# cliangyu/video-diffusion

Measured on AMD Instinct MI355X. Metric: denoise-steps/sec, higher is better.
Workload: dtype f32

## Files before the change

include/vd_amd.h:

```cpp
#ifndef VD_AMD_H
#define VD_AMD_H
#ifdef __cplusplus
extern "C" {
#endif

typedef struct vd_config {
    int image_size;
    int num_channels;
    int num_res_blocks;
    int num_heads;
    int T;
    int n_attention_ds;
    int attention_ds[8];
    int use_scale_shift_norm;
    int use_spatial_encoding;
    int use_frame_encoding;
    int enforce_position_invariance;
    int use_rpe_net;
    int allow_interactions_between_padding;
    float rp_alpha, rp_beta, rp_gamma;
    int time_embed_mult;
    int cond_emb_type;
    int learn_sigma;
} vd_config;
// ... 141 lines not shown
int vd_op_conv_split(const float* src0, int Cin, int nfr, int Hs, int Ws, int stride, const void* w_split, const float* bias,
                     const float* res, float* out, int Cout, void* stream);
int vd_pack_conv3_wino_split(const float* host_oihw, unsigned short* host_out, int O, int I);
int vd_op_conv_wino_split(const float* src0, int Cin, int nfr, int Hs, int Ws, int ups, const void* w_split, const float* bias,
                          const float* res, const float* fbias, int fbias_ld, float* out, int Cout, double* gn_part,
                          void* stream);
int vd_op_conv_wino_act(const float* src0, const float* src1, int C0, int Cin, int nfr, int Hs, int Ws, const void* w_split, const float* bias,
                        const float* affA, const float* affB, const float* res, float* out, int Cout, double* gn_part, void* stream);
int vd_conv_wino_act_ok(int nfr, int H, int Cin, int Cout);
int vd_pack_conv3_wino_ups(const float* host_oihw, unsigned short* host_out, int O, int I);
int vd_conv_ups_stats_split(int Hs);
int vd_op_conv_wino_ups(const float* src0, int Cin, int nfr, int Hs, const void* w_ups, const float* bias, float* out, int Cout,
                        double* gn_part, void* stream);
int vd_op_linear_split(const float* a, int M, int K, const void* w_split, const float* bias, const float* res, int act,
                       float* out, int N, void* stream);
int vd_op_linear_split_stats(const float* a, int M, int K, const void* w_split, const float* bias, const float* res, int act,
                             float* out, int N, int HW, double* gn_part, void* stream);
int vd_linear_stats_split(int M, int N, int HW);
int vd_op_gn_fold(const float* src0, const float* src1, int C0, int C, int nfr, int HW, const float* gamma,
                  const float* beta, const float* film, int film_ld, float* affA, float* affB, void* stream);
int vd_op_affine_apply(const float* x, const float* affA, const float* affB, int nfr, int HW, int C, float* y,
                       void* stream);
int vd_op_affine_act(const float* src0, const float* src1, int C0, int C, const float* affA, const float* affB, int nfr,
                     int HW, int act, float* y, void* stream);
int vd_op_gn_temporal(const float* x, const float* gamma, const float* beta, int B, int T, int HW, int C, float* y,
                      void* stream);
int vd_op_attn_spatial(const float* qkv, int nfr, int L, int C, int heads, float* out, void* stream);
int vd_op_attn_temporal(const float* qkv, const float* Rk, const float* Rq, const float* Rv, const float* mask, int B,
                        int T, int HW, int C, int heads, int allow_pad, float* out, void* stream);
int vd_op_out_conv(const float* x, const float* affA, const float* affB, const float* w_packed, const float* bias,
// ... 59 lines not shown
```

video-diffusion_amd/_lib.py:

```python
import ctypes
import os
import subprocess

_HERE = os.path.dirname(os.path.abspath(__file__))
_CSRC = os.path.join(_HERE, "csrc")
SO_PATH = os.path.join(_HERE, "libvdamd.so")
SOURCES = ["igemm.hip", "conv_wino.hip", "conv_wino_r64.hip", "conv_wino_z128.hip", "gemm_frag.hip", "gemm_split.hip", "split_pack.hip", "norm.hip", "backward.hip", "attn_spatial.hip", "attn_temporal.hip", "attn_temporal_long.hip", "misc.hip", "engine.hip", "lpips.hip", "metrics.hip", "i3d.hip", "conv_cl.hip", "hallway.hip"]
HEADER = os.path.join(os.path.dirname(_HERE), "include", "vd_amd.h")
HEADERS = [os.path.join(_CSRC, "vd_common.h"), os.path.join(_CSRC, "wino_common.h"), os.path.join(_CSRC, "igemm_tile.h"), HEADER]
SOURCE_FLAGS = {"conv_wino_z128.hip": ["-mllvm", "-pragma-unroll-threshold=1000000"]}


def _toolchain():
    hipcc = os.environ.get("HIPCC", "/opt/rocm/bin/hipcc")
    flags = ["--offload-arch=gfx950", "-O3", "-std=c++17", "-fPIC", "-Wno-unused-value"] + \
        os.environ.get("VD_HIPCC_FLAGS", "").split()
    return hipcc, flags


def _sha(*parts):
    import hashlib
    h = hashlib.sha1()
    for p in parts:
        h.update(p if isinstance(p, bytes) else str(p).encode())
# ... 157 lines not shown
    "vd_pack_linear_frag": (_I, [_P, _P, _I, _I]),
    "vd_pack_linear_split": (_I, [_P, _P, _I, _I]),
    "vd_pack_conv3_wino_split": (_I, [_P, _P, _I, _I]),
    "vd_set_model_mean_type": (_I, [_P, _I]),
    "vd_math_mode": (_I, []),
    "vd_split_image_u16": (_L, [_L, _L]),
    "vd_pack_conv3_wino_ups": (_I, [_P, _P, _I, _I]),
    "vd_conv_ups_stats_split": (_I, [_I]),
    "vd_op_conv_wino_ups": (_I, [_P, _I, _I, _I, _P, _P, _P, _I, _P, _P]),
    "vd_op_conv_wino_split": (_I, [_P, _I, _I, _I, _I, _I, _P, _P, _P, _P, _I, _P, _I, _P, _P]),
    "vd_op_conv_wino_act": (_I, [_P, _P, _I, _I, _I, _I, _I, _P, _P, _P, _P, _P, _P, _I, _P, _P]),
    "vd_conv_wino_act_ok": (_I, [_I, _I, _I, _I]),
    "vd_pack_conv3_split": (_I, [_P, _P, _I, _I]),
    "vd_op_conv_split": (_I, [_P, _I, _I, _I, _I, _I, _P, _P, _P, _P, _I, _P]),
    "vd_op_linear_split": (_I, [_P, _I, _I, _P, _P, _P, _I, _P, _I, _P]),
    "vd_op_linear_split_stats": (_I, [_P, _I, _I, _P, _P, _P, _I, _P, _I, _I, _P, _P]),
    "vd_linear_stats_split": (_I, [_I, _I, _I]),
    "vd_op_gn_fold": (_I, [_P, _P, _I, _I, _I, _I, _P, _P, _P, _I, _P, _P, _P]),
    "vd_op_affine_apply": (_I, [_P, _P, _P, _I, _I, _I, _P, _P]),
    "vd_op_affine_act": (_I, [_P, _P, _I, _I, _P, _P, _I, _I, _I, _P, _P]),
    "vd_op_gn_temporal": (_I, [_P, _P, _P, _I, _I, _I, _I, _P, _P]),
    "vd_op_attn_spatial": (_I, [_P, _I, _I, _I, _I, _P, _P]),
    "vd_op_attn_temporal": (_I, [_P, _P, _P, _P, _P, _I, _I, _I, _I, _I, _I, _P, _P]),
    "vd_op_out_conv": (_I, [_P, _P, _P, _P, _P, _I, _I, _I, _I, _I, _P, _P]),
    "vd_op_gn_bwd": (_I, [_P, _P, _I, _I, _P, _P, _P, _P, _I, _I, _I, _P, _P, _I, _P, _I, _P]),
    "vd_op_gn_temporal_bwd": (_I, [_P, _P, _P, _I, _I, _I, _I, _I, _P, _P]),
    "vd_op_attn_temporal_bwd": (_I, [_P, _P, _P, _P, _P, _I, _I, _I, _I, _I, _I, _P, _P, _P]),
    "vd_op_attn_spatial_bwd": (_I, [_P, _I, _I, _I, _I, _P, _P, _P]),
    "vd_op_out_conv_bwd": (_I, [_P, _P, _I, _I, _I, _I, _I, _P, _P]),
    "vd_op_stem_col2im": (_I, [_P, _P, _P, _P, _I, _I, _I, _I, _P, _P]),
# ... 73 lines not shown
```

video-diffusion_amd/csrc/engine.hip:

```cpp
#include <cmath>
#include <cstring>
#include <unordered_map>
#include <vector>

#include "../../include/vd_amd.h"
#include "vd_common.h"

namespace vd {

thread_local std::string g_last_error;
void set_error(const std::string& msg) { g_last_error = msg; }

int launch_frame_t(const int64_t* fidx, int B, int T, int center, float* tv, hipStream_t s);

enum ParamKind { PK_RAW = 0, PK_CONV3, PK_STEM, PK_POSENC, PK_OUTCONV, PK_LINF, PK_CONV3W, PK_CONV3S,
                 PK_CONV3WU };

struct Param {
    std::string name;
    int nd = 0;
    long long shape[4] = {1, 1, 1, 1};
    size_t numel = 0;
    size_t packed = 0;
    size_t off = 0;
// ... 21 lines not shown
struct TapeConv { int type, idx; Tens in, out; };
struct TapePos { Tens in, out; };
struct TapeOp { int kind, i; };
struct Tape {
    std::vector<TapeOp> ops;
    std::vector<TapeRes> res; std::vector<TapeAttn> attn; std::vector<TapeConv> conv; std::vector<TapePos> pos;
    Tens head; float *headA = nullptr, *headB = nullptr, *head_mr = nullptr;
    void clear() { ops.clear(); res.clear(); attn.clear(); conv.clear(); pos.clear(); }
};

static const int CH_MULT_256[] = {1, 1, 2, 2, 4, 4};
static const int CH_MULT_128[] = {1, 1, 2, 3, 4};
static const int CH_MULT_64[] = {1, 2, 3, 4};
static const int CH_MULT_32[] = {1, 2, 2, 2};
static bool split_math() { return math_mode() != MATH_FP32; }

constexpr int STEM_KPAD = 64;

struct Arena {
    char* base = nullptr;
    size_t cap = 0, used = 0, peak = 0;
    bool dry = false, overflow = false;
    template <class Tp> Tp* get(size_t n) {
        size_t bytes = (n * sizeof(Tp) + 255) & ~(size_t)255;
        if (!dry && cap && used + bytes > cap) {
            overflow = true;
            return reinterpret_cast<Tp*>(base);
        }
        char* p = (dry ? reinterpret_cast<char*>(0x1000) : base) + used;
        used += bytes;
// ... 44 lines not shown
};
struct ProfPause {
    bool was = g_prof.on;
    ProfPause() { g_prof.on = false; }
    ~ProfPause() { g_prof.on = was; }
};

static bool act_conv_will_dispatch(const IgemmArgs& g) {
    return g.affA && igemm_kernel(igemm_first_launch(g)) == IK_Z128;
}

static int igemm_p(const IgemmArgs& g, hipStream_t st, int cin_alg = 0) {
    const double taps = (double)g.ksz * g.ksz, cin = cin_alg ? cin_alg : g.Cin;
    const double in_pix = (double)g.nfr * g.Hs * g.Ws;
    const double nz = g.zcount > 1 ? g.zcount : 1;
    const double bytes = nz * 4.0 * (in_pix * cin + (double)g.M * g.Cout * (g.res ? 2 : 1) + taps * cin * g.Cout + (g.side ? in_pix * cin : 0.0));
    const IgemmArgs one = igemm_first_launch(g);
    const IgemmKernel k = igemm_kernel(one);
    const bool wino = k == IK_R64_UPS || k == IK_Z128 || k == IK_R64 || k == IK_WINO;
    const int tile = igemm_tile_class(igemm_sel_M(one), g.Cout);
    int cls;
    switch (k) {
        case IK_R64_UPS: cls = PC_CONV_WINO_R64_UPS; break;
        case IK_Z128: cls = PC_CONV_WINO_Z128; break;
        case IK_R64: cls = PC_CONV_WINO_R64; break;
        case IK_WINO: cls = PC_CONV_WINO; break;
        case IK_SPLIT: cls = gemm_split_tile_class(igemm_sel_M(one), g.Cout) == 4 ? (int)PC_IGEMM_128x192 : tile; break;
        default: cls = tile + (g.ksz == 3 ? (int)PC_CONV_128x128 : 0);
    }
    char tag[56];
    snprintf(tag, sizeof(tag), "M=%d N=%d K=%d k%d s%d%s%s%s", g.M, g.Cout, g.Cin, g.ksz, g.stride, g.ups ? " ups" : "",
             g.affA ? " pro" : (g.act ? " act" : ""), g.res ? " res" : "");
    VD_REQUIRE(g.stats == nullptr || wino || (k == IK_SPLIT && g.stats_hw > 0),
               "GroupNorm partial sums requested from a kernel that has no such epilogue");
    ProfScope ps(cls, nz * 2.0 * g.M * g.Cout * cin * taps, bytes, st, tag);
    return launch_igemm(g, st);
}

static int affine_act(const float* src0, const float* src1, int C0, int C, const float* A, const float* B, int N, int HW,
                      float* y, hipStream_t st) {
    ProfScope ps(PC_ELEMENTWISE, 0.0, 8.0 * N * HW * C, st);
    return launch_affine_act(src0, src1, C0, C, A, B, N, HW, 1, y, st);
}

struct FwdIn {
    int B, T;
    const float *x, *obs_src, *obs, *lat, *km, *t_model;
// ... 511 lines not shown
    const int H = x0.H, HW = H * H;
    const int cin = x0.C + (x1 ? x1->C : 0);
    VD_REQUIRE(cin == r.cin, "ResBlock input channels");
    const float* s1 = x1 ? x1->p : nullptr;
    float *A1 = nullptr, *B1 = nullptr, *A2 = nullptr, *B2 = nullptr, *mr1 = nullptr, *mr2 = nullptr;
    int rc;
    const float* film = film_all + r.film_off;
    IgemmArgs gsk{};
    bool fuse_skip = false;
    if (r.skw >= 0) {
        gsk = conv_args(x0, x1, N, 1, 1, 0);
        set_w(gsk, r.skw); gsk.Cout = r.cout; gsk.ldo = r.cout; gsk.side_hw = HW;
        IgemmArgs one = gsk; one.nfr = std::max(1, std::min(N, igemm_frames_per_launch(gsk)));
        one.M = (g_sel_nfr ? std::max(g_sel_nfr, one.nfr) : one.nfr) * HW;
        one.wfrag = one.wfrag ? one.wfrag : reinterpret_cast<const float*>(0x1000);
        fuse_skip = params[r.skw].kind == PK_LINF && split_math() && gemm_split_side_supported(one);
    }
    const bool fold = !tape;
    const int nsel = g_sel_nfr > N ? g_sel_nfr : N;
    const bool za1 = !tape && params[r.c1w].kind == PK_CONV3W && f16_math() && x0.C % 16 == 0 && conv_wino_z128_act_shape(nsel, H, cin, r.cout);
    if (za1 && !ar.dry) fuse_skip = false;
    const bool fold1 = fold && !fuse_skip;
    const bool za2 = !tape && params[r.c2w].kind == PK_CONV3W && f16_math() && conv_wino_z128_act_shape(nsel, H, r.cout, r.cout);
    if ((!fold1 || za1 || ar.dry) && (rc = gn_fold(x0, x1, N, r.gn1w, r.gn1b, nullptr, 0, st, ar, &A1, &B1, &mr1))) return rc;
    float* h = ar.get<float>((size_t)N * HW * r.cout);
    Tens ht{h, r.cout, H};
    if (params[r.c1w].kind == PK_CONV3W) ht.part = stats_table(ar, N, H, r.cout, &ht.split);
    Tens ot{nullptr, r.cout, H};
    if (params[r.c2w].kind == PK_CONV3W) ot.part = stats_table(ar, N, H, r.cout, &ot.split);
    float* sk_early = fuse_skip ? ar.get<float>((size_t)N * HW * r.cout) : nullptr;
    {
// ... 92 lines not shown
        if (!cfg.use_rpe_net)
            for (int i = 0; i < 3; ++i)
                if ((rc = launch_rpe_table(W(rp[i]->table), fidx, B, T, C, cfg.rp_alpha, cfg.rp_beta, cfg.rp_gamma,
                                           Rall + i * rrows * C, st))) return rc;
        AttnTemporalArgs ta{qkv, R[0], R[1], R[2], amask, o, B, T, HW, C, cfg.num_heads,
                            cfg.allow_interactions_between_padding, scale};
        { const double Fd = C / cfg.num_heads;
          ProfScope ps(PC_ATTN_TEMPORAL, 10.0 * B * HW * cfg.num_heads * T * T * Fd, 16.0 * tok * C + 12.0 * rrows * C, st);
          rc = launch_attn_temporal(ta, st); }
        if (rc) return rc;
        if (!attn_cap_t.empty() && attn_seq < (int)attn_cap_t.size() && attn_cap_t[attn_seq] &&
            (rc = launch_attn_temporal_weights(ta, attn_cap_t[attn_seq], st))) return rc;
        if ((rc = linear(o, (int)tok, C, C, W(a.tp.projw), W(a.tp.projb), 0, xn, xt, st, &xt_t))) return rc;
    }
    float *A = nullptr, *Bf = nullptr, *mrs = nullptr;
    const bool fold = !tape;
    if (!fold && (rc = gn_fold(xt_t, nullptr, N, a.sp.normw, a.sp.normb, nullptr, 0, st, ar, &A, &Bf, &mrs))) return rc;
    float* xn2 = ar.get<float>(tok * C);
    float* qkv2 = ar.get<float>(tok * 3 * C);
    float* o2 = ar.get<float>(tok * C);
    float* xs = ar.get<float>(tok * C);
    Tens xs_t{xs, C, H};
    gemm_stats_table(ar, (int)tok, C, C, &xs_t);
    if (fold && (rc = gn_act(xt_t, nullptr, N, a.sp.normw, a.sp.normb, nullptr, 0, 0, xn2, st, ar))) return rc;
    if (!ar.dry) {
        if (!fold) { ProfScope ps(PC_ELEMENTWISE, 0.0, 8.0 * tok * C, st); rc = launch_affine_apply(xt, A, Bf, N, HW, C, xn2, st); }
        if (rc) return rc;
        if ((rc = linear(xn2, (int)tok, C, 3 * C, W(a.sp.qkvw), W(a.sp.qkvb), 0, nullptr, qkv2, st))) return rc;
        AttnSpatialArgs sa{qkv2, o2, N, HW, C, cfg.num_heads, scale};
        { ProfScope ps(PC_ATTN_SPATIAL, 4.0 * N * (double)HW * HW * C, 16.0 * tok * C, st); rc = launch_attn_spatial(sa, st); }
        if (rc) return rc;
        if (!attn_cap_s.empty() && attn_seq < (int)attn_cap_s.size() && attn_cap_s[attn_seq] &&
            (rc = launch_attn_spatial_weights(sa, attn_cap_s[attn_seq], st))) return rc;
        if ((rc = linear(o2, (int)tok, C, C, W(a.sp.projw), W(a.sp.projb), 0, xn2, xs, st, &xs_t))) return rc;
    }
    *out = xs_t;
    if (!ar.dry) ++attn_seq;
    if (tape) {
        tape->ops.push_back(TapeOp{2, (int)tape->attn.size()});
        tape->attn.push_back(TapeAttn{(int)(&a - attn.data()), x, B, T, xn, qkv, R[0], R[1], R[2], o, xt, A, Bf, mrs, xn2, qkv2, o2, xs, amask});
    }
    return 0;
}

void vd_engine::rpe_group_blocks() {
    if (!rpe_groups.empty()) return;
    for (size_t b = 0; b < attn.size(); ++b) {
        size_t gi = 0;
        while (gi < rpe_groups.size() && rpe_groups[gi].C != attn[b].C) ++gi;
// ... 1339 lines not shown
}

int vd_pack_linear_split(const float* host_w, unsigned short* host_out, int N, int K) {
    VD_REQUIRE(host_w && host_out && N % 32 == 0 && K % 32 == 0, "vd_pack_linear_split: N, K multiples of 32");
    pack_linear_split(host_w, host_out, N, K, N, 0);
    return 0;
}

int vd_op_linear_split(const float* a, int M, int K, const void* w_split, const float* bias, const float* res, int act,
                       float* out, int N, void* stream) {
    IgemmArgs g = linear_args(M, K, N);
    g.src0 = a; g.wfrag = static_cast<const float*>(w_split); g.wsplit = 1; g.bias = bias; g.act = act; g.res = res; g.out = out;
    return launch_igemm(g, static_cast<hipStream_t>(stream));
}

int vd_op_linear_split_stats(const float* a, int M, int K, const void* w_split, const float* bias, const float* res, int act,
                             float* out, int N, int HW, double* gn_part, void* stream) {
    IgemmArgs g = linear_args(M, K, N);
    g.src0 = a; g.wfrag = static_cast<const float*>(w_split); g.wsplit = 1; g.bias = bias; g.act = act; g.res = res; g.out = out;
    VD_REQUIRE(gn_part && HW > 0 && gemm_split_supported(g), "vd_op_linear_split_stats: shape not covered by gemm_split.hip");
    g.stats = gn_part; g.stats_hw = HW; g.stats_split = HW / gemm_split_stats_rows(M, N);
    return launch_igemm(g, static_cast<hipStream_t>(stream));
}

int vd_linear_stats_split(int M, int N, int HW) { return HW / gemm_split_stats_rows(M, N); }

int vd_pack_conv3_wino(const float* host_oihw, float* host_out, int O, int I) {
    VD_REQUIRE(host_oihw && host_out && O % 64 == 0 && I % 16 == 0, "O multiple of 64, I multiple of 16");
    pack_conv3_wino(host_oihw, host_out, O, I);
    return 0;
// ... 206 lines not shown
```

video-diffusion_amd/csrc/gemm_split.hip:

```cpp
#include <cstring>
#include <vector>

#include "vd_common.h"

namespace vd {

typedef __bf16 bf16x4 __attribute__((ext_vector_type(4)));
typedef __bf16 bf16x8 __attribute__((ext_vector_type(8)));
typedef unsigned u32x4 __attribute__((ext_vector_type(4)));
typedef unsigned u32x2 __attribute__((ext_vector_type(2)));

template <bool F16>
__device__ __forceinline__ f32x16 mfma_piece(u32x4 a, u32x4 b, f32x16 c) {
    if constexpr (F16) return __builtin_amdgcn_mfma_f32_32x32x16_f16(__builtin_bit_cast(f16x8, a), __builtin_bit_cast(f16x8, b), c, 0, 0, 0);
    else return __builtin_amdgcn_mfma_f32_32x32x16_bf16(__builtin_bit_cast(bf16x8, a), __builtin_bit_cast(bf16x8, b), c, 0, 0, 0);
}

#ifndef VD_GS_SKIP
#define VD_GS_SKIP 0
#endif
#ifdef VD_GS_TIMING
__device__ unsigned long long g_gs_stamp[8];
#define GS_STAMP(i) do { if (threadIdx.x == 0 && blockIdx.x == gridDim.x / 2 && blockIdx.y == 0) {                        \
        __builtin_amdgcn_sched_barrier(0); g_gs_stamp[i] = __builtin_amdgcn_s_memrealtime(); __builtin_amdgcn_sched_barrier(0); } } while (0)
// ... 8 lines not shown
    if constexpr (F16) {
        p1.x = f16_pack(v.x, v.y); p1.y = f16_pack(v.z, v.w);
        p2.x = f16_pack_scaled(f16_rem_lo(p1.x, v.x), f16_rem_hi(p1.x, v.y));
        p2.y = f16_pack_scaled(f16_rem_lo(p1.y, v.z), f16_rem_hi(p1.y, v.w));
        p3 = p2;
    } else {
        const bf16x4 q1 = __builtin_convertvector(v, bf16x4);
        f32x4 r = v - __builtin_convertvector(q1, f32x4);
        const bf16x4 q2 = __builtin_convertvector(r, bf16x4);
        r = r - __builtin_convertvector(q2, f32x4);
        const bf16x4 q3 = __builtin_convertvector(r, bf16x4);
        p1 = __builtin_bit_cast(u32x2, q1); p2 = __builtin_bit_cast(u32x2, q2); p3 = __builtin_bit_cast(u32x2, q3);
    }
}

template <int BM, int BN, bool ACT, bool CONV, bool F16 = true, bool SIDE = false>
__global__ __launch_bounds__(256, 2) void gemm_split_kernel(IgemmArgs a) {
    constexpr int MI = BM / 64, NI = BN / 64, AR = BM / 32;
    constexpr bool B2R = F16;
    constexpr int RING = NI >= 3 ? 2 : (BM == 64 && BN == 64) ? 6 : 3;
    constexpr int BP = B2R ? 2 : 3;
    constexpr int PF = BM == 64 ? 3 : 1;
    constexpr int NPL = F16 ? 2 : 3;
    constexpr int PLANE = BM * SROW, ABUF = NPL * PLANE;
    extern __shared__ __attribute__((aligned(16))) char smem_c[];
    const int tid = threadIdx.x, lane = tid & 63, wave = __builtin_amdgcn_readfirstlane(tid >> 6);
    GS_STAMP(0);
    const int wm = wave >> 1, wn = wave & 1;
    const int lr = lane & 31, lh = lane >> 5;
    int bxi = blockIdx.x, byi = blockIdx.y;
    if (gridDim.y > 1 && (gridDim.x & 7) == 0 && gridDim.x >= 128) {
// ... 28 lines not shown
            iy0[j] = (int)oy * a.stride - 1;
            ix0[j] = (int)ox * a.stride - 1;
            ao0[j] = (unsigned)(((int)n * a.Hs + iy0[j]) * a.Ws + ix0[j]) * (unsigned)(a.Cin * 4) + lq * 16u;
            ao1[j] = 0;
        } else {
            ao0[j] = row * (unsigned)(a.C0 * 4) + lq * 16u;
            ao1[j] = row * (unsigned)(C1 * 4) + lq * 16u;
        }
    }
    const auto bsrc = __builtin_amdgcn_make_buffer_rsrc(const_cast<float*>(a.wfrag), 0, (CONV ? 9 : 1) * a.Cin * a.Cout * 6, 0x00020000);
    unsigned bo[NI];
#pragma unroll
    for (int j = 0; j < NI; ++j) bo[j] = (unsigned)min(byi * (BN / 32) + wn * NI + j, ncoblk - 1) * 3072u + lane * 16u;

    f32x4 ra[PF][AR];
    u32x4 bfr[RING][NI][BP], b2[NI], afr[2][MI][NPL];
    static_assert(!SIDE || (BM == 128 && !CONV && !ACT), "side output: 128-row tiles of a plain 1x1");
    const bool side_on = SIDE && byi == 0;
    const float* sAp = SIDE ? a.sideA + (size_t)(m0 / (SIDE ? a.side_hw : 1)) * a.Cin + lq * 4 : nullptr;
    const float* sBp = SIDE ? a.sideB + (size_t)(m0 / (SIDE ? a.side_hw : 1)) * a.Cin + lq * 4 : nullptr;
    f32x4 sA = {0.f, 0.f, 0.f, 0.f}, sB = sA;
    auto side_affine = [&](int chunk) {
        if constexpr (SIDE) {
            if (side_on) { sA = *reinterpret_cast<const f32x4*>(sAp + chunk * 32); sB = *reinterpret_cast<const f32x4*>(sBp + chunk * 32); }
        }
    };
    auto side_store = [&](f32x4 v, int chunk, int j) {
        if constexpr (SIDE) {
            const int row = m0 + lrow + 32 * j;
            if (side_on && row < a.M) {
                f32x4 r = v * sA + sB;
                r.x = silu_f(r.x); r.y = silu_f(r.y); r.z = silu_f(r.z); r.w = silu_f(r.w);
// ... 11 lines not shown
                const bool ok = (unsigned)(iy0[j] + kh) < (unsigned)a.Hs && (unsigned)(ix0[j] + kw) < (unsigned)a.Ws;
                ra[rs][j] = __builtin_bit_cast(f32x4, __builtin_amdgcn_raw_buffer_load_b128(asrc0, ok ? ao0[j] + shift : 0x80000000u, c * 4, 0));
            }
            return;
        }
        const int c = chunk * 32;
        if (c < a.C0) {
#pragma unroll
            for (int j = 0; j < AR; ++j)
                ra[rs][j] = __builtin_bit_cast(f32x4, __builtin_amdgcn_raw_buffer_load_b128(asrc0, ao0[j], c * 4, 0));
        } else {
#pragma unroll
            for (int j = 0; j < AR; ++j)
                ra[rs][j] = __builtin_bit_cast(f32x4, __builtin_amdgcn_raw_buffer_load_b128(asrc1, ao1[j], (c - a.C0) * 4, 0));
        }
    };
    auto a_store = [&](char* Ad, int rs) {
#pragma unroll
        for (int j = 0; j < AR; ++j) {
            f32x4 v = ra[rs][j];
            side_store(v, 0, j);
            if constexpr (ACT) { v.x = silu_f(v.x); v.y = silu_f(v.y); v.z = silu_f(v.z); v.w = silu_f(v.w); }
            u32x2 p1, p2, p3;
            split3<F16>(v, p1, p2, p3);
            char* d = Ad + (lrow + 32 * j) * SROW + lq * 8;
            *reinterpret_cast<u32x2*>(d) = p1;
            *reinterpret_cast<u32x2*>(d + PLANE) = p2;
            if constexpr (!F16) *reinterpret_cast<u32x2*>(d + 2 * PLANE) = p3;
        }
    };
    const unsigned two_m12 = 0x0c000c00u;
    auto b_third = [&](int slot, int j) {
        if constexpr (B2R)
            asm("v_pk_mul_f16 %0, %4, %8\n\tv_pk_mul_f16 %1, %5, %8\n\tv_pk_mul_f16 %2, %6, %8\n\tv_pk_mul_f16 %3, %7, %8"
                : "=&v"(b2[j][0]), "=&v"(b2[j][1]), "=&v"(b2[j][2]), "=&v"(b2[j][3])
                : "v"(bfr[slot][j][0][0]), "v"(bfr[slot][j][0][1]), "v"(bfr[slot][j][0][2]), "v"(bfr[slot][j][0][3]), "s"(two_m12));
// ... 27 lines not shown
        bv[j] = a.bias && co < a.Cout ? a.bias[co] : 0.f;
        wsc[j] = F16 ? trailer[min(co, a.Cout - 1)] : 1.f;
        winv[j] = F16 ? trailer[a.Cout + min(co, a.Cout - 1)] : 1.f;
#pragma unroll
        for (int i = 0; i < MI; ++i)
            vb[i][j] = co < a.Cout ? (unsigned)((m0 + wm * (BM / 2) + i * 32 + 4 * lh) * a.ldo + co) * 4u : 0x80000000u;
    }
    f32x16 acc[MI][NI];
#pragma unroll
    for (int i = 0; i < MI; ++i)
#pragma unroll
        for (int j = 0; j < NI; ++j)
#pragma unroll
            for (int r = 0; r < 16; ++r) acc[i][j][r] = bv[j];
    if (a.res) {
#pragma unroll
        for (int i = 0; i < MI; ++i)
#pragma unroll
            for (int j = 0; j < NI; ++j)
#pragma unroll
                for (int r = 0; r < 16; ++r) {
                    const int srow = ((r & 3) + 8 * (r >> 2)) * a.ldo * 4;
                    acc[i][j][r] += __builtin_bit_cast(float, __builtin_amdgcn_raw_buffer_load_b32(rsrc, vb[i][j] + srow, 0, 0));
                }
    }
    if constexpr (F16) {
#pragma unroll
        for (int i = 0; i < MI; ++i)
#pragma unroll
            for (int j = 0; j < NI; ++j)
#pragma unroll
                for (int r = 0; r < 16; ++r) acc[i][j][r] *= wsc[j];
    }

    const int nks = 2 * nchunk;
    a_prefetch(0, 0);
    side_affine(0);
    if constexpr (PF == 3) { a_prefetch(min(1, nchunk - 1), 1); a_prefetch(min(2, nchunk - 1), 2); }
// ... 8 lines not shown
        const int j = idx / 3, p2 = idx - 3 * j;
        if (p2 >= BP) return;
        bfr[slot][j][p2] = __builtin_bit_cast(u32x4, __builtin_amdgcn_raw_buffer_load_b128(bsrc, bo[j] + p2 * 1024, kstep * ncoblk * 3072, 0));
    };
    auto a_prefetch_one = [&](int chunk, int rs, int j) {
        if constexpr (CONV) {
            const int tap = chunk / cpt, c = (chunk - tap * cpt) * 32;
            const int kh = tap / 3, kw = tap - 3 * kh;
            const unsigned shift = (unsigned)((kh * a.Ws + kw) * a.Cin * 4);
            const bool ok = (unsigned)(iy0[j] + kh) < (unsigned)a.Hs && (unsigned)(ix0[j] + kw) < (unsigned)a.Ws;
            ra[rs][j] = __builtin_bit_cast(f32x4, __builtin_amdgcn_raw_buffer_load_b128(asrc0, ok ? ao0[j] + shift : 0x80000000u, c * 4, 0));
        } else {
            const int c = chunk * 32;
            ra[rs][j] = c < a.C0 ? __builtin_bit_cast(f32x4, __builtin_amdgcn_raw_buffer_load_b128(asrc0, ao0[j], c * 4, 0))
                                 : __builtin_bit_cast(f32x4, __builtin_amdgcn_raw_buffer_load_b128(asrc1, ao1[j], (c - a.C0) * 4, 0));
        }
    };
    auto a_frag_one = [&](int slot, const char* Ab, int ks, int idx) {
        const int i = idx / 3, p2 = idx - 3 * i;
        if (p2 >= NPL) return;
        afr[slot][i][p2] = *reinterpret_cast<const u32x4*>(Ab + p2 * PLANE + aoff + i * 32 * SROW + ks * 32);
    };
    auto a_store_one = [&](char* Ad, int rs, int j, int data_chunk) {
        f32x4 v = ra[rs][j];
        if (data_chunk >= 0) side_store(v, data_chunk, j);
        if constexpr (ACT) { v.x = silu_f(v.x); v.y = silu_f(v.y); v.z = silu_f(v.z); v.w = silu_f(v.w); }
        u32x2 p1, p2, p3;
        if (VD_GS_SKIP & 8) {
            p1 = u32x2{__builtin_bit_cast(unsigned, v.x), __builtin_bit_cast(unsigned, v.y)};
            p2 = u32x2{__builtin_bit_cast(unsigned, v.z), __builtin_bit_cast(unsigned, v.w)};
            p3 = p2;
        } else split3<F16>(v, p1, p2, p3);
        char* d = Ad + (lrow + 32 * j) * SROW + lq * 8;
        *reinterpret_cast<u32x2*>(d) = p1;
        *reinterpret_cast<u32x2*>(d + PLANE) = p2;
        if constexpr (!F16) *reinterpret_cast<u32x2*>(d + 2 * PLANE) = p3;
    };
    constexpr int NT = MI * NI;
    auto kstep = [&](int chunk, int ks, int gslot, int aslot, int pf_chunk, int pf_slot, int st_slot) {
        const int g = 2 * chunk + ks;
// ... 101 lines not shown


bool conv_split_supported(const IgemmArgs& a) {
    return a.wsplit && a.wfrag != nullptr && a.ksz == 3 && a.pad == 1 && (a.stride == 1 || a.stride == 2) && a.ups == 0 &&
           a.Cout % 32 == 0 && a.Cin % 32 == 0 && a.C0 == a.Cin && a.affA == nullptr && a.fbias == nullptr && a.zcount <= 1 &&
           (a.res == nullptr || a.res_ld == a.ldo) && (size_t)a.nfr * a.Hs * a.Ws * a.Cin < (1u << 28) &&
           (size_t)a.M * a.ldo < (1u << 28) && (size_t)9 * a.Cin * a.Cout * 6 < (1u << 31);
}

bool gemm_split_supported(const IgemmArgs& a) {
    return a.wsplit && a.wfrag != nullptr && a.ksz == 1 && a.stride == 1 && a.pad == 0 && a.ups == 0 && a.Cout % 32 == 0 &&
           a.Cin % 32 == 0 && a.C0 % 32 == 0 && a.affA == nullptr && a.fbias == nullptr && (a.res == nullptr || a.res_ld == a.ldo) &&
           (size_t)a.M * std::max(std::max(a.C0, a.Cin - a.C0), a.ldo) < (1u << 28) && (size_t)a.Cin * a.Cout * 6 < (1u << 31);
}

bool gemm_split_side_supported(const IgemmArgs& a) {
    return gemm_split_supported(a) && a.act == 0 && a.zcount <= 1 && gemm_split_tile_class(igemm_sel_M(a), a.Cout) == 0 &&
           a.side_hw > 0 && a.side_hw % 128 == 0 && a.M % a.side_hw == 0;
}

template <int BM, int BN, bool F16>
static int launch_gs_m(const IgemmArgs& a, hipStream_t s) {
    const size_t lds = (size_t)2 * (F16 ? 2 : 3) * BM * SROW;
    dim3 grid((a.M + BM - 1) / BM, (a.Cout + BN - 1) / BN, a.zcount > 1 ? a.zcount : 1);
    if (a.side) {
        if constexpr (BM == 128 && BN == 128) {
            VD_REQUIRE(gemm_split_side_supported(a) && a.sideA && a.sideB, "side output: plain 1x1 on the 128x128 tile, whole frames of a multiple of 128 rows");
            hipLaunchKernelGGL((gemm_split_kernel<128, 128, false, false, F16, true>), grid, dim3(256), lds, s, a);
            VD_HIP(hipGetLastError());
            return 0;
        } else {
            VD_REQUIRE(false, "side output: 128x128 tile only");
        }
    }
    if (a.ksz == 3) {
        if (a.act) hipLaunchKernelGGL((gemm_split_kernel<BM, BN, true, true, F16>), grid, dim3(256), lds, s, a);
        else hipLaunchKernelGGL((gemm_split_kernel<BM, BN, false, true, F16>), grid, dim3(256), lds, s, a);
    } else if (a.act) hipLaunchKernelGGL((gemm_split_kernel<BM, BN, true, false, F16>), grid, dim3(256), lds, s, a);
    else hipLaunchKernelGGL((gemm_split_kernel<BM, BN, false, false, F16>), grid, dim3(256), lds, s, a);
    VD_HIP(hipGetLastError());
    return 0;
}
template <int BM, int BN>
static int launch_gs(const IgemmArgs& a, hipStream_t s) {
    return f16_math() ? launch_gs_m<BM, BN, true>(a, s) : launch_gs_m<BM, BN, false>(a, s);
}

int gemm_split_tile_class(int M, int Cout) {
    const int base = igemm_tile_class(M, Cout);
    if (base != 0 || Cout % 192) return base;
    return (long)((M + 127) / 128) * (Cout / 192) >= 384 ? 4 : base;
}

int gemm_split_stats_rows(int M, int Cout) {
    const int c = gemm_split_tile_class(M, Cout);
    return c == 2 || c == 3 ? 32 : 64;
}

int launch_gemm_split(const IgemmArgs& a, int tile_class, hipStream_t s) {
    if (tile_class == 0) tile_class = gemm_split_tile_class(igemm_sel_M(a), a.Cout);
    if (a.stats) {
        const int rows = tile_class == 2 || tile_class == 3 ? 32 : 64;
        VD_REQUIRE(a.zcount <= 1 && a.stats_hw > 0 && a.stats_hw % rows == 0 && a.M % a.stats_hw == 0 &&
                   a.stats_split == a.stats_hw / rows, "GroupNorm partial sums from the GEMM epilogue: whole frames of a multiple of the wave tile's rows");
    }
    switch (tile_class) {
        case 4: return launch_gs<128, 192>(a, s);
        case 0: return launch_gs<128, 128>(a, s);
        case 1: return launch_gs<128, 64>(a, s);
        case 2: return launch_gs<64, 128>(a, s);
        default: return launch_gs<64, 64>(a, s);
    }
}

}
// ... 1 lines not shown
```

video-diffusion_amd/csrc/igemm.hip:

```cpp
#include <algorithm>

#include <string>

#include "igemm_tile.h"
#include "vd_common.h"

namespace vd {

constexpr int BK = IG_BK;
constexpr int LDP = IG_LDP;

template <int BM, int BN>
__global__ __launch_bounds__(256) void igemm_kernel(IgemmArgs a) {
    constexpr int MI = BM / 64, NI = BN / 64;
    constexpr int AR = BM / 32, BR = BN / 32;
    extern __shared__ __attribute__((aligned(16))) float smem[];
    float* As = smem;
    float* Bs = smem + 2 * BM * LDP;

    const int tid = threadIdx.x, lane = tid & 63, wave = tid >> 6;
    const int wm = wave >> 1, wn = wave & 1;
    const int lr = lane & 31;
    const int m0 = blockIdx.x * BM, n0 = blockIdx.y * BN;

// ... 97 lines not shown
}

IgemmKernel igemm_kernel(const IgemmArgs& a) {
    if (a.ups_phase) return IK_R64_UPS;
    if (gemm_split_supported(a) || conv_split_supported(a)) return IK_SPLIT;
    if (conv_wino_z128_act_supported(a) || conv_wino_z128_supported(a)) return IK_Z128;
    if (conv_wino_r64_supported(a)) return IK_R64;
    if (gemm_frag_supported(a)) return IK_FRAG;
    if (conv_wino_supported(a)) return IK_WINO;
    return IK_GENERIC;
}

static int launch_igemm_one(const IgemmArgs& a, hipStream_t s) {
    const IgemmKernel k = igemm_kernel(a);
    const int tile = igemm_tile_class(igemm_sel_M(a), a.Cout);
    switch (k) {
        case IK_R64_UPS:
            VD_REQUIRE(conv_wino_r64_supported(a), "sub-pixel Upsample conv: shape not covered by conv_wino_r64.hip");
            return launch_conv_wino_r64(a, s);
        case IK_SPLIT: return launch_gemm_split(a, tile, s);
        case IK_Z128: return launch_conv_wino_z128(a, s);
        case IK_R64: return launch_conv_wino_r64(a, s);
        case IK_FRAG: return launch_gemm_frag(a, tile, s);
        case IK_WINO: return launch_conv_wino(a, s);
        case IK_GENERIC: break;
    }
    VD_REQUIRE(!a.wsplit, "split weight image given for a shape the split kernels do not cover");
    VD_REQUIRE(a.w != nullptr, "this shape runs on the generic kernel and needs [tap][Cout][Cin] weights");
    switch (tile) {
        case 0: return launch_t<128, 128>(a, s);
// ... 72 lines not shown
```

video-diffusion_amd/csrc/vd_common.h:

```cpp
#pragma once
#include <hip/hip_runtime.h>
#include <cstdint>
#include <cstdio>
#include <string>

typedef float f32x4 __attribute__((ext_vector_type(4)));
typedef float f32x16 __attribute__((ext_vector_type(16)));

namespace vd {

constexpr int kMaxWindowFrames = 128;
constexpr int kMaxGuidedWindowFrames = 32;

void set_error(const std::string& msg);
extern thread_local std::string g_last_error;

#define VD_HIP(call)                                                                   \
    do {                                                                               \
        hipError_t e_ = (call);                                                        \
        if (e_ != hipSuccess) {                                                        \
            vd::set_error(std::string(#call) + ": " + hipGetErrorString(e_));          \
            return -2;                                                                 \
        }                                                                              \
    } while (0)
// ... 65 lines not shown
    const float* res;
    int res_ld;
    const float* fbias;
    int fbias_ld;
    float* out;
    int ldo;
    int Cout, M;
    double* stats;
    int stats_split;
    int stats_hw;
    int zcount, zs_a, zs_out;
    const long long* ztab = nullptr; const float* zbase = nullptr;
    int wsplit;
    float* ksplit_ws;
    size_t ksplit_ws_floats;
};

struct AttnSpatialArgs {
    const float* qkv;
    float* out;
    int nfr, L, C, heads;
    float scale;
};

struct AttnTemporalArgs {
    const float* qkv;
    const float* Rk;
    const float* Rq;
    const float* Rv;
    const float* mask;
// ... 93 lines not shown
}
size_t split_image_u16(size_t n_out, size_t k_total);
void pack_conv3_wino_split(const float* oihw, unsigned short* out, int O, int I);
bool conv_wino_r64_supported(const IgemmArgs& a);
int launch_conv_wino_r64(const IgemmArgs& a, hipStream_t s);
bool conv_wino_z128_supported(const IgemmArgs& a);
bool conv_wino_z128_shape(int nfr, int H, int Cin, int Cout);
int launch_conv_wino_z128(const IgemmArgs& a, hipStream_t s);
bool conv_wino_z128_act_shape(int nfr, int H, int Cin, int Cout);
bool conv_wino_z128_act_supported(const IgemmArgs& a);
void pack_conv3_wino_ups(const float* oihw, unsigned short* out, int O, int I);
int conv_wino_ups_stats_split(int Hs);
int conv_wino_r64_ksplit(int nfr, int Hl, int Cin, int Cout);
size_t conv_wino_r64_ksplit_floats(int nfr, int Hl, int Cin, int Cout, int nfr_sel = 0);
bool gemm_split_supported(const IgemmArgs& a);
bool gemm_split_side_supported(const IgemmArgs& a);
bool conv_split_supported(const IgemmArgs& a);
void pack_conv3_split(const float* w_oihw, unsigned short* out, int Cout, int Cin);
int launch_gemm_split(const IgemmArgs& a, int tile_class, hipStream_t s);
int gemm_split_tile_class(int M, int Cout);
int gemm_split_stats_rows(int M, int Cout);
void pack_linear_split(const float* w, unsigned short* out_base, int rows, int K, int n_total, int row0);
int launch_conv_wino(const IgemmArgs& a, hipStream_t s);
void pack_conv3_wino(const float* oihw, float* out, int O, int I);
int launch_attn_spatial(const AttnSpatialArgs& a, hipStream_t s);
int launch_attn_temporal(const AttnTemporalArgs& a, hipStream_t s);
int launch_attn_temporal_long(const AttnTemporalArgs& a, hipStream_t s);

int launch_gn_stats(const float* src0, const float* src1, int C0, int C, int nfr, int HW, double* part, int split,
                    hipStream_t s);
int gn_stats_split(int nfr, int HW, int C);
// ... 160 lines not shown
```

Before: 51.27.

## Fuse GroupNorm affine into split-GEMM prologue for spatial attention qkv/proj

Adds a PRE variant of the split GEMM kernel that applies the per-frame GroupNorm affine (A*x+B) to the activation tile as it is loaded. It also applies the same affine to the residual in the epilogue. Spatial attention now feeds raw activations to the qkv and proj GEMMs, so the separate affine_apply pass and the normalized intermediate buffer are no longer needed. The skip side-output path is also generalized to tile classes beyond 128x128. The cost is extra per-tile loads of the affine coefficients and more registers in the GEMM kernel.

```diff
diff --git a/include/vd_amd.h b/include/vd_amd.h
--- a/include/vd_amd.h
+++ b/include/vd_amd.h
@@ -179,6 +179,11 @@
                         double* gn_part, void* stream);
 int vd_op_linear_split(const float* a, int M, int K, const void* w_split, const float* bias, const float* res, int act,
                        float* out, int N, void* stream);
+int vd_op_linear_split_pre(const float* a, int M, int K, const void* w_split, const float* bias, const float* res, const float* preA,
+                           const float* preB, int pre_hw, int res_affine, float* out, int N, int tile_class, void* stream);
+int vd_op_linear_split_side(const float* a0, const float* a1, int C0, int M, int K, const void* w_split, const float* bias,
+                            const float* sideA, const float* sideB, int side_hw, float* out, float* side_out, int N, int tile_class,
+                            void* stream);
 int vd_op_linear_split_stats(const float* a, int M, int K, const void* w_split, const float* bias, const float* res, int act,
                              float* out, int N, int HW, double* gn_part, void* stream);
 int vd_linear_stats_split(int M, int N, int HW);
diff --git a/video-diffusion_amd/_lib.py b/video-diffusion_amd/_lib.py
--- a/video-diffusion_amd/_lib.py
+++ b/video-diffusion_amd/_lib.py
@@ -195,6 +195,8 @@
     "vd_pack_conv3_split": (_I, [_P, _P, _I, _I]),
     "vd_op_conv_split": (_I, [_P, _I, _I, _I, _I, _I, _P, _P, _P, _P, _I, _P]),
     "vd_op_linear_split": (_I, [_P, _I, _I, _P, _P, _P, _I, _P, _I, _P]),
+    "vd_op_linear_split_pre": (_I, [_P, _I, _I, _P, _P, _P, _P, _P, _I, _I, _P, _I, _I, _P]),
+    "vd_op_linear_split_side": (_I, [_P, _P, _I, _I, _I, _P, _P, _P, _P, _I, _P, _P, _I, _I, _P]),
     "vd_op_linear_split_stats": (_I, [_P, _I, _I, _P, _P, _P, _I, _P, _I, _I, _P, _P]),
     "vd_linear_stats_split": (_I, [_I, _I, _I]),
     "vd_op_gn_fold": (_I, [_P, _P, _I, _I, _I, _I, _P, _P, _P, _I, _P, _P, _P]),
diff --git a/video-diffusion_amd/csrc/engine.hip b/video-diffusion_amd/csrc/engine.hip
--- a/video-diffusion_amd/csrc/engine.hip
+++ b/video-diffusion_amd/csrc/engine.hip
@@ -59,6 +59,10 @@
 static const int CH_MULT_64[] = {1, 2, 3, 4};
 static const int CH_MULT_32[] = {1, 2, 2, 2};
 static bool split_math() { return math_mode() != MATH_FP32; }
+
+#ifndef VD_NORM_IN_GEMM
+#define VD_NORM_IN_GEMM 3
+#endif
 
 constexpr int STEM_KPAD = 64;
 
@@ -133,7 +137,8 @@
     const double taps = (double)g.ksz * g.ksz, cin = cin_alg ? cin_alg : g.Cin;
     const double in_pix = (double)g.nfr * g.Hs * g.Ws;
     const double nz = g.zcount > 1 ? g.zcount : 1;
-    const double bytes = nz * 4.0 * (in_pix * cin + (double)g.M * g.Cout * (g.res ? 2 : 1) + taps * cin * g.Cout + (g.side ? in_pix * cin : 0.0));
+    const double bytes = nz * 4.0 * (in_pix * cin + (double)g.M * g.Cout * (g.res ? 2 : 1) + taps * cin * g.Cout + (g.side ? in_pix * cin : 0.0) +
+                                     (g.preA ? 2.0 * (g.M / g.pre_hw) * cin : 0.0));
     const IgemmArgs one = igemm_first_launch(g);
     const IgemmKernel k = igemm_kernel(one);
     const bool wino = k == IK_R64_UPS || k == IK_Z128 || k == IK_R64 || k == IK_WINO;
@@ -149,7 +154,7 @@
     }
     char tag[56];
     snprintf(tag, sizeof(tag), "M=%d N=%d K=%d k%d s%d%s%s%s", g.M, g.Cout, g.Cin, g.ksz, g.stride, g.ups ? " ups" : "",
-             g.affA ? " pro" : (g.act ? " act" : ""), g.res ? " res" : "");
+             g.affA ? " pro" : (g.preA ? " pre" : (g.act ? " act" : "")), g.res ? " res" : "");
     VD_REQUIRE(g.stats == nullptr || wino || (k == IK_SPLIT && g.stats_hw > 0),
                "GroupNorm partial sums requested from a kernel that has no such epilogue");
     ProfScope ps(cls, nz * 2.0 * g.M * g.Cout * cin * taps, bytes, st, tag);
@@ -691,7 +696,8 @@
         IgemmArgs one = gsk; one.nfr = std::max(1, std::min(N, igemm_frames_per_launch(gsk)));
         one.M = (g_sel_nfr ? std::max(g_sel_nfr, one.nfr) : one.nfr) * HW;
         one.wfrag = one.wfrag ? one.wfrag : reinterpret_cast<const float*>(0x1000);
-        fuse_skip = params[r.skw].kind == PK_LINF && split_math() && gemm_split_side_supported(one);
+        fuse_skip = params[r.skw].kind == PK_LINF && split_math() && gemm_split_side_supported(one) &&
+                    ((VD_NORM_IN_GEMM & 2) || gemm_split_tile_class(igemm_sel_M(one), one.Cout) == 0);
     }
     const bool fold = !tape;
     const int nsel = g_sel_nfr > N ? g_sel_nfr : N;
@@ -814,9 +820,13 @@
         if ((rc = linear(o, (int)tok, C, C, W(a.tp.projw), W(a.tp.projb), 0, xn, xt, st, &xt_t))) return rc;
     }
     float *A = nullptr, *Bf = nullptr, *mrs = nullptr;
-    const bool fold = !tape;
+    IgemmArgs gq = linear_args((int)tok, C, 3 * C), gp = linear_args((int)tok, C, C);
+    gq.pre_hw = gp.pre_hw = HW; gp.res_affine = 1;
+    gq.wfrag = gp.wfrag = reinterpret_cast<const float*>(this);
+    const bool pre = (VD_NORM_IN_GEMM & 1) && !tape && split_math() && gemm_split_pre_supported(gq) && gemm_split_pre_supported(gp);
+    const bool fold = !tape && !pre;
     if (!fold && (rc = gn_fold(xt_t, nullptr, N, a.sp.normw, a.sp.normb, nullptr, 0, st, ar, &A, &Bf, &mrs))) return rc;
-    float* xn2 = ar.get<float>(tok * C);
+    float* xn2 = pre ? nullptr : ar.get<float>(tok * C);
     float* qkv2 = ar.get<float>(tok * 3 * C);
     float* o2 = ar.get<float>(tok * C);
     float* xs = ar.get<float>(tok * C);
@@ -824,15 +834,24 @@
     gemm_stats_table(ar, (int)tok, C, C, &xs_t);
     if (fold && (rc = gn_act(xt_t, nullptr, N, a.sp.normw, a.sp.normb, nullptr, 0, 0, xn2, st, ar))) return rc;
     if (!ar.dry) {
-        if (!fold) { ProfScope ps(PC_ELEMENTWISE, 0.0, 8.0 * tok * C, st); rc = launch_affine_apply(xt, A, Bf, N, HW, C, xn2, st); }
+        if (!fold && !pre) { ProfScope ps(PC_ELEMENTWISE, 0.0, 8.0 * tok * C, st); rc = launch_affine_apply(xt, A, Bf, N, HW, C, xn2, st); }
         if (rc) return rc;
-        if ((rc = linear(xn2, (int)tok, C, 3 * C, W(a.sp.qkvw), W(a.sp.qkvb), 0, nullptr, qkv2, st))) return rc;
+        if (pre) {
+            gq.src0 = xt; gq.preA = A; gq.preB = Bf; gq.wfrag = W(a.sp.qkvw); gq.bias = W(a.sp.qkvb); gq.out = qkv2;
+            rc = igemm_p(gq, st);
+        } else rc = linear(xn2, (int)tok, C, 3 * C, W(a.sp.qkvw), W(a.sp.qkvb), 0, nullptr, qkv2, st);
+        if (rc) return rc;
         AttnSpatialArgs sa{qkv2, o2, N, HW, C, cfg.num_heads, scale};
         { ProfScope ps(PC_ATTN_SPATIAL, 4.0 * N * (double)HW * HW * C, 16.0 * tok * C, st); rc = launch_attn_spatial(sa, st); }
         if (rc) return rc;
         if (!attn_cap_s.empty() && attn_seq < (int)attn_cap_s.size() && attn_cap_s[attn_seq] &&
             (rc = launch_attn_spatial_weights(sa, attn_cap_s[attn_seq], st))) return rc;
-        if ((rc = linear(o2, (int)tok, C, C, W(a.sp.projw), W(a.sp.projb), 0, xn2, xs, st, &xs_t))) return rc;
+        if (pre) {
+            gp.src0 = o2; gp.preA = A; gp.preB = Bf; gp.res = xt; gp.wfrag = W(a.sp.projw); gp.bias = W(a.sp.projb); gp.out = xs;
+            if (xs_t.part) { gp.stats = xs_t.part; gp.stats_split = xs_t.split; gp.stats_hw = HW; }
+            rc = igemm_p(gp, st);
+        } else rc = linear(o2, (int)tok, C, C, W(a.sp.projw), W(a.sp.projb), 0, xn2, xs, st, &xs_t);
+        if (rc) return rc;
     }
     *out = xs_t;
     if (!ar.dry) ++attn_seq;
@@ -2202,6 +2221,27 @@
     return launch_igemm(g, static_cast<hipStream_t>(stream));
 }
 
+int vd_op_linear_split_pre(const float* a, int M, int K, const void* w_split, const float* bias, const float* res, const float* preA,
+                           const float* preB, int pre_hw, int res_affine, float* out, int N, int tile_class, void* stream) {
+    IgemmArgs g = linear_args(M, K, N);
+    g.src0 = a; g.wfrag = static_cast<const float*>(w_split); g.wsplit = 1; g.bias = bias; g.res = res; g.out = out;
+    g.preA = preA; g.preB = preB; g.pre_hw = pre_hw; g.res_affine = res_affine; g.tile_force = tile_class;
+    VD_REQUIRE(split_math() && preA && preB && tile_class >= 0 && tile_class <= 4 && (!res_affine || res) && gemm_split_pre_supported(g),
+               "vd_op_linear_split_pre: shape not covered by gemm_split.hip's affine prologue");
+    return launch_igemm(g, static_cast<hipStream_t>(stream));
+}
+
+int vd_op_linear_split_side(const float* a0, const float* a1, int C0, int M, int K, const void* w_split, const float* bias,
+                            const float* sideA, const float* sideB, int side_hw, float* out, float* side_out, int N, int tile_class,
+                            void* stream) {
+    IgemmArgs g = linear_args(M, K, N);
+    g.src0 = a0; g.src1 = a1; g.C0 = C0; g.wfrag = static_cast<const float*>(w_split); g.wsplit = 1; g.bias = bias; g.out = out;
+    g.side = side_out; g.sideA = sideA; g.sideB = sideB; g.side_hw = side_hw; g.tile_force = tile_class;
+    VD_REQUIRE(split_math() && side_out && sideA && sideB && tile_class >= 0 && tile_class <= 4 && igemm_frames_per_launch(g) >= M &&
+               gemm_split_side_supported(g, tile_class), "vd_op_linear_split_side: shape not covered by gemm_split.hip's side output");
+    return launch_igemm(g, static_cast<hipStream_t>(stream));
+}
+
 int vd_op_linear_split_stats(const float* a, int M, int K, const void* w_split, const float* bias, const float* res, int act,
                              float* out, int N, int HW, double* gn_part, void* stream) {
     IgemmArgs g = linear_args(M, K, N);
diff --git a/video-diffusion_amd/csrc/gemm_split.hip b/video-diffusion_amd/csrc/gemm_split.hip
--- a/video-diffusion_amd/csrc/gemm_split.hip
+++ b/video-diffusion_amd/csrc/gemm_split.hip
@@ -46,7 +46,7 @@
     }
 }
 
-template <int BM, int BN, bool ACT, bool CONV, bool F16 = true, bool SIDE = false>
+template <int BM, int BN, bool ACT, bool CONV, bool F16 = true, bool SIDE = false, bool PRE = false>
 __global__ __launch_bounds__(256, 2) void gemm_split_kernel(IgemmArgs a) {
     constexpr int MI = BM / 64, NI = BN / 64, AR = BM / 32;
     constexpr bool B2R = F16;
@@ -105,8 +105,25 @@
     for (int j = 0; j < NI; ++j) bo[j] = (unsigned)min(byi * (BN / 32) + wn * NI + j, ncoblk - 1) * 3072u + lane * 16u;
 
     f32x4 ra[PF][AR];
+    static_assert(!PRE || (!CONV && !ACT && !SIDE), "affine prologue: plain 1x1");
+    constexpr int NH = BM / 64;
+    f32x4 pA[PRE ? PF : 1][NH], pB[PRE ? PF : 1][NH];
+    const int npre = PRE ? (a.M / (PRE ? a.pre_hw : 1)) * a.Cin * 4 : 0;
+    const auto pasrc = __builtin_amdgcn_make_buffer_rsrc(const_cast<float*>(PRE ? a.preA : a.src0), 0, npre, 0x00020000);
+    const auto pbsrc = __builtin_amdgcn_make_buffer_rsrc(const_cast<float*>(PRE ? a.preB : a.src0), 0, npre, 0x00020000);
+    unsigned po[NH];
+    if constexpr (PRE) {
+#pragma unroll
+        for (int h = 0; h < NH; ++h) po[h] = ((unsigned)(min(m0 + 64 * h, a.M - 1) / a.pre_hw) * (unsigned)a.Cin + lq * 4u) * 4u;
+    }
+    auto pre_load = [&](int chunk, int rs, int h) {
+        if constexpr (PRE) {
+            pA[rs][h] = __builtin_bit_cast(f32x4, __builtin_amdgcn_raw_buffer_load_b128(pasrc, po[h], chunk * 128, 0));
+            pB[rs][h] = __builtin_bit_cast(f32x4, __builtin_amdgcn_raw_buffer_load_b128(pbsrc, po[h], chunk * 128, 0));
+        }
+    };
     u32x4 bfr[RING][NI][BP], b2[NI], afr[2][MI][NPL];
-    static_assert(!SIDE || (BM == 128 && !CONV && !ACT), "side output: 128-row tiles of a plain 1x1");
+    static_assert(!SIDE || (!CONV && !ACT), "side output: a plain 1x1");
     const bool side_on = SIDE && byi == 0;
     const float* sAp = SIDE ? a.sideA + (size_t)(m0 / (SIDE ? a.side_hw : 1)) * a.Cin + lq * 4 : nullptr;
     const float* sBp = SIDE ? a.sideB + (size_t)(m0 / (SIDE ? a.side_hw : 1)) * a.Cin + lq * 4 : nullptr;
@@ -148,12 +165,15 @@
             for (int j = 0; j < AR; ++j)
                 ra[rs][j] = __builtin_bit_cast(f32x4, __builtin_amdgcn_raw_buffer_load_b128(asrc1, ao1[j], (c - a.C0) * 4, 0));
         }
+#pragma unroll
+        for (int h = 0; h < NH; ++h) pre_load(chunk, rs, h);
     };
     auto a_store = [&](char* Ad, int rs) {
 #pragma unroll
         for (int j = 0; j < AR; ++j) {
             f32x4 v = ra[rs][j];
             side_store(v, 0, j);
+            if constexpr (PRE) v = v * pA[rs][j >> 1] + pB[rs][j >> 1];
             if constexpr (ACT) { v.x = silu_f(v.x); v.y = silu_f(v.y); v.z = silu_f(v.z); v.w = silu_f(v.w); }
             u32x2 p1, p2, p3;
             split3<F16>(v, p1, p2, p3);
@@ -211,6 +231,18 @@
 #pragma unroll
             for (int r = 0; r < 16; ++r) acc[i][j][r] = bv[j];
     if (a.res) {
+        float rA[NI], rB[NI];
+        const bool raff = PRE && a.res_affine;
+        if constexpr (PRE) {
+            if (raff) {
+                const unsigned fo = (unsigned)(min(m0 + wm * (BM / 2), a.M - 1) / a.pre_hw) * (unsigned)a.Cin;
+#pragma unroll
+                for (int j = 0; j < NI; ++j) {
+                    const unsigned co = (unsigned)min(n0 + wn * (BN / 2) + j * 32 + lr, a.Cout - 1);
+                    rA[j] = a.preA[fo + co]; rB[j] = a.preB[fo + co];
+                }
+            }
+        }
 #pragma unroll
         for (int i = 0; i < MI; ++i)
 #pragma unroll
@@ -218,7 +250,9 @@
 #pragma unroll
                 for (int r = 0; r < 16; ++r) {
                     const int srow = ((r & 3) + 8 * (r >> 2)) * a.ldo * 4;
-                    acc[i][j][r] += __builtin_bit_cast(float, __builtin_amdgcn_raw_buffer_load_b32(rsrc, vb[i][j] + srow, 0, 0));
+                    float rv = __builtin_bit_cast(float, __builtin_amdgcn_raw_buffer_load_b32(rsrc, vb[i][j] + srow, 0, 0));
+                    if constexpr (PRE) { if (raff) rv = __builtin_fmaf(rv, rA[j], rB[j]); }
+                    acc[i][j][r] += rv;
                 }
     }
     if constexpr (F16) {
@@ -257,6 +291,7 @@
             const int c = chunk * 32;
             ra[rs][j] = c < a.C0 ? __builtin_bit_cast(f32x4, __builtin_amdgcn_raw_buffer_load_b128(asrc0, ao0[j], c * 4, 0))
                                  : __builtin_bit_cast(f32x4, __builtin_amdgcn_raw_buffer_load_b128(asrc1, ao1[j], (c - a.C0) * 4, 0));
+            if ((j & 1) == 0) pre_load(chunk, rs, j >> 1);
         }
     };
     auto a_frag_one = [&](int slot, const char* Ab, int ks, int idx) {
@@ -267,6 +302,7 @@
     auto a_store_one = [&](char* Ad, int rs, int j, int data_chunk) {
         f32x4 v = ra[rs][j];
         if (data_chunk >= 0) side_store(v, data_chunk, j);
+        if constexpr (PRE) v = v * pA[rs][j >> 1] + pB[rs][j >> 1];
         if constexpr (ACT) { v.x = silu_f(v.x); v.y = silu_f(v.y); v.z = silu_f(v.z); v.w = silu_f(v.w); }
         u32x2 p1, p2, p3;
         if (VD_GS_SKIP & 8) {
@@ -398,9 +434,18 @@
            (size_t)a.M * std::max(std::max(a.C0, a.Cin - a.C0), a.ldo) < (1u << 28) && (size_t)a.Cin * a.Cout * 6 < (1u << 31);
 }
 
-bool gemm_split_side_supported(const IgemmArgs& a) {
-    return gemm_split_supported(a) && a.act == 0 && a.zcount <= 1 && gemm_split_tile_class(igemm_sel_M(a), a.Cout) == 0 &&
-           a.side_hw > 0 && a.side_hw % 128 == 0 && a.M % a.side_hw == 0;
+static int tile_class_rows(int tile_class) { return tile_class == 2 || tile_class == 3 ? 64 : 128; }
+
+bool gemm_split_side_supported(const IgemmArgs& a, int tile_class) {
+    if (tile_class < 0) tile_class = gemm_split_tile_class(igemm_sel_M(a), a.Cout);
+    return gemm_split_supported(a) && a.act == 0 && a.zcount <= 1 && a.side_hw > 0 && a.side_hw % tile_class_rows(tile_class) == 0 &&
+           a.M % a.side_hw == 0;
+}
+
+bool gemm_split_pre_supported(const IgemmArgs& a) {
+    return gemm_split_supported(a) && a.act == 0 && a.zcount <= 1 && a.src1 == nullptr && a.C0 == a.Cin && a.side == nullptr &&
+           a.pre_hw > 0 && a.pre_hw % 64 == 0 && a.M % a.pre_hw == 0 && igemm_frames_per_launch(a) >= a.nfr &&
+           (!a.res_affine || a.Cin == a.Cout);
 }
 
 template <int BM, int BN, bool F16>
@@ -408,14 +453,17 @@
     const size_t lds = (size_t)2 * (F16 ? 2 : 3) * BM * SROW;
     dim3 grid((a.M + BM - 1) / BM, (a.Cout + BN - 1) / BN, a.zcount > 1 ? a.zcount : 1);
     if (a.side) {
-        if constexpr (BM == 128 && BN == 128) {
-            VD_REQUIRE(gemm_split_side_supported(a) && a.sideA && a.sideB, "side output: plain 1x1 on the 128x128 tile, whole frames of a multiple of 128 rows");
-            hipLaunchKernelGGL((gemm_split_kernel<128, 128, false, false, F16, true>), grid, dim3(256), lds, s, a);
-            VD_HIP(hipGetLastError());
-            return 0;
-        } else {
-            VD_REQUIRE(false, "side output: 128x128 tile only");
-        }
+        VD_REQUIRE(!a.preA && gemm_split_supported(a) && a.act == 0 && a.zcount <= 1 && a.side_hw > 0 && a.side_hw % BM == 0 && a.M % a.side_hw == 0 &&
+                   a.sideA && a.sideB, "side output: plain 1x1, whole frames of a multiple of the tile's rows");
+        hipLaunchKernelGGL((gemm_split_kernel<BM, BN, false, false, F16, true>), grid, dim3(256), lds, s, a);
+        VD_HIP(hipGetLastError());
+        return 0;
+    }
+    if (a.preA) {
+        VD_REQUIRE(gemm_split_pre_supported(a) && a.preB, "affine prologue: plain 1x1 over one source, whole frames of a multiple of 64 rows, one launch");
+        hipLaunchKernelGGL((gemm_split_kernel<BM, BN, false, false, F16, false, true>), grid, dim3(256), lds, s, a);
+        VD_HIP(hipGetLastError());
+        return 0;
     }
     if (a.ksz == 3) {
         if (a.act) hipLaunchKernelGGL((gemm_split_kernel<BM, BN, true, true, F16>), grid, dim3(256), lds, s, a);
@@ -442,7 +490,8 @@
 }
 
 int launch_gemm_split(const IgemmArgs& a, int tile_class, hipStream_t s) {
-    if (tile_class == 0) tile_class = gemm_split_tile_class(igemm_sel_M(a), a.Cout);
+    if (a.tile_force >= 0) tile_class = a.tile_force;
+    else if (tile_class == 0) tile_class = gemm_split_tile_class(igemm_sel_M(a), a.Cout);
     if (a.stats) {
         const int rows = tile_class == 2 || tile_class == 3 ? 32 : 64;
         VD_REQUIRE(a.zcount <= 1 && a.stats_hw > 0 && a.stats_hw % rows == 0 && a.M % a.stats_hw == 0 &&
diff --git a/video-diffusion_amd/csrc/igemm.hip b/video-diffusion_amd/csrc/igemm.hip
--- a/video-diffusion_amd/csrc/igemm.hip
+++ b/video-diffusion_amd/csrc/igemm.hip
@@ -135,6 +135,7 @@
 static int launch_igemm_one(const IgemmArgs& a, hipStream_t s) {
     const IgemmKernel k = igemm_kernel(a);
     const int tile = igemm_tile_class(igemm_sel_M(a), a.Cout);
+    VD_REQUIRE((!a.preA && !a.side) || k == IK_SPLIT, "affine prologue / side output: gemm_split.hip only");
     switch (k) {
         case IK_R64_UPS:
             VD_REQUIRE(conv_wino_r64_supported(a), "sub-pixel Upsample conv: shape not covered by conv_wino_r64.hip");
diff --git a/video-diffusion_amd/csrc/vd_common.h b/video-diffusion_amd/csrc/vd_common.h
--- a/video-diffusion_amd/csrc/vd_common.h
+++ b/video-diffusion_amd/csrc/vd_common.h
@@ -103,6 +103,8 @@
     int wsplit;
     float* ksplit_ws;
     size_t ksplit_ws_floats;
+    const float* preA = nullptr; const float* preB = nullptr; int pre_hw = 0; int res_affine = 0;
+    int tile_force = -1;
 };
 
 struct AttnSpatialArgs {
@@ -226,7 +228,8 @@
 int conv_wino_r64_ksplit(int nfr, int Hl, int Cin, int Cout);
 size_t conv_wino_r64_ksplit_floats(int nfr, int Hl, int Cin, int Cout, int nfr_sel = 0);
 bool gemm_split_supported(const IgemmArgs& a);
-bool gemm_split_side_supported(const IgemmArgs& a);
+bool gemm_split_pre_supported(const IgemmArgs& a);
+bool gemm_split_side_supported(const IgemmArgs& a, int tile_class = -1);
 bool conv_split_supported(const IgemmArgs& a);
 void pack_conv3_split(const float* w_oihw, unsigned short* out, int Cout, int Cin);
 int launch_gemm_split(const IgemmArgs& a, int tile_class, hipStream_t s);
```

After: 51.37, median of 6. No clear change (+0.2%).
